# jfc4050/detect-to-track

Measured on AMD Instinct MI355X. Metric: PointwiseCorrelation fwd+bwd Gvox/s (and % HBM roofline) at B=8 C=256 38×63 d=8, higher is better.
Workload: dtype f32

## Files before the change

### detect-to-track_amd/csrc/d2t_corr_bwd8.hip

```cpp
#include "d2t_corr_common.hpp"
#include <type_traits>

namespace d2t { namespace tuned {

#ifdef D2T_LAB
__device__ unsigned long long* lab8_stamps;
#define D2T_WCLK(var) do { __builtin_amdgcn_sched_barrier(0); asm volatile("s_memtime %0\n\ts_waitcnt lgkmcnt(0)" : "=s"(var)::"memory"); __builtin_amdgcn_sched_barrier(0); } while (0)
#define D2T_WRT(var) do { __builtin_amdgcn_sched_barrier(0); asm volatile("s_memrealtime %0\n\ts_waitcnt lgkmcnt(0)" : "=s"(var)::"memory"); __builtin_amdgcn_sched_barrier(0); } while (0)
#define D2T_LAB_ONLY(...) __VA_ARGS__
#else
#define D2T_WCLK(var)
#define D2T_WRT(var)
#define D2T_LAB_ONLY(...)
#endif

namespace {

constexpr int S8_CH = 256;
constexpr int S8_QUADS = KB_SS * NACT * 64;
constexpr int S8_RING = 2048 * 4;
constexpr int S8_OOR = 0x7ffffff0;

struct Quad8 { int off, info; };

template <bool ROWKB>
__device__ __forceinline__ void kb_slot(int q, int gg, int& xr, int& cg)
{
    if (ROWKB) {
        xr = q < 4 ? q : gg;
        cg = q < 4 ? gg : 4;
    } else {
        const int x = 4 * q + gg;
        xr = (x * 13) >> 6;
        cg = x - xr * NCG;
    }
}

template <bool ROWKB>
__device__ __forceinline__ Quad8 quad8_desc(int role, int e, int H, int W, int tiles_i, int j0, int col0)
{
    const int q = e / (NACT * 64), r = e - q * (NACT * 64);
    const int a = r >> 6, l = r & 63, gg = l >> 4;
    int xr, cg;
    kb_slot<ROWKB>(q < KB_SS ? q : 0, gg, xr, cg);
    const int tpi = (l >> 2) & 3, lo2 = l & 3;
    const int ci = role ? 4 * a + tpi - xr : xr - 4 * a - tpi + 2 * DT;
    const int tj = j0 + lo2, sj = col0 + 4 * cg + (role ? lo2 : 0);
    const int cj = role ? j0 - sj + DT : sj - tj + DT;
    int mask = 0;
#pragma unroll
    for (int c = 0; c < 4; ++c) {
        const bool col_ok = role ? j0 + c < W : tj < W;
        mask |= (cj + c >= 0 && cj + c < 2 * DT && col_ok) ? (1 << c) : 0;
    }
    if (ci < 0 || ci >= 2 * DT || e >= S8_QUADS) mask = 0;
    const int pix0 = role ? xr * W + sj : (4 * (a - 2) + tpi) * W + tj;
    int lo = 2 - a, hi = tiles_i + 2 - a;
    const int hi_t = (H - tpi + 3) / 4 + 2 - a;
    const int hi_r = (H - xr + 3) / 4;
    hi = hi < hi_t ? hi : hi_t;
    hi = hi < hi_r ? hi : hi_r;
    lo = lo < 0 ? 0 : lo;
    if (!mask || hi < lo) { lo = 0; hi = 0; }
    Quad8 d;
    d.off = (pix0 * CELLS + ci * CW + cj) * 4;
    d.info = lo | (hi << 8) | (mask << 16);
    return d;
}

__device__ __forceinline__ f32x4 quad8_fix(const f32x4& v, int info)
{
    const u32x4 b = __builtin_bit_cast(u32x4, v);
    u32x4 o;
#pragma unroll
    for (int c = 0; c < 4; ++c) o[c] = b[c] & (unsigned)__builtin_amdgcn_sbfe(info, 16 + c, 1);
    return __builtin_bit_cast(f32x4, o);
}

typedef std::integral_constant<int, 0> I0;
typedef std::integral_constant<int, 1> I1;
typedef std::integral_constant<int, 2> I2;
typedef std::integral_constant<int, 3> I3;
typedef std::integral_constant<int, 4> I4;
typedef std::integral_constant<int, 5> I5;

#define D2T_PIN() __builtin_amdgcn_sched_barrier(0)

#ifndef D2T_EXP_GCO
#define D2T_EXP_GCO 1
#endif
#ifndef D2T_EXP_SWZ
#define D2T_EXP_SWZ 1
#endif
#ifndef D2T_EXP_PRIO
#define D2T_EXP_PRIO 0
#endif
#ifndef S8_ABL
#define S8_ABL 0
#endif
template <int role, int S8_CT, bool ROWKB, int ABL = 0, bool FLEX = false>
__device__ __forceinline__ void strip8_body(float (&ring)[2][S8_RING], const float* __restrict__ gout,
                                            const float* __restrict__ fm0, const float* __restrict__ fm1,
                                            float* __restrict__ g0, float* __restrict__ g1,
                                            int b, int tj, int C, int H, int W, int tiles_i, int ct0, int nct)
{
    constexpr int S8_WAVES = 16 / S8_CT;
    constexpr int GT = S8_WAVES * 64, S8_NQ = 2048 / GT;
    constexpr int DEAD0 = ROWKB ? 3 : KB_SS - 1;
    const int tid = threadIdx.x, lane = tid & 63, n = lane & 15, g = lane >> 4;
    const int wave = __builtin_amdgcn_readfirstlane(tid >> 6);
    D2T_LAB_ONLY(unsigned long long w_t0, w_t1, w_t2, w_t3, w_r1, w_r2, w_a, w_b, w_sl[3] = {0, 0, 0}, w_bar = 0, w_rot = 0;)
    D2T_WCLK(w_t0);
    const int j0 = tj * TP, HW = H * W;
    const int wleft = j0 - DT + role;
    const int col0 = wleft < 0 ? 0 : (wleft > W - WC ? W - WC : wleft);
    const float* S = (role ? fm0 : fm1) + (size_t)b * C * HW;
    float* gx = (role ? g1 : g0) + (size_t)b * C * HW;
    const float* gb = gout + (size_t)b * HW * CELLS;
    const unsigned plane_bytes = (unsigned)C * HW * 4u;
    const __amdgpu_buffer_rsrc_t rs = uniform_rsrc(S, plane_bytes);
    const __amdgpu_buffer_rsrc_t rx = uniform_rsrc(gx, plane_bytes);
    const __amdgpu_buffer_rsrc_t rg = uniform_rsrc(gb, (unsigned)HW * CELLS * 4u);

    const int cw = FLEX ? (ct0 + wave) * 16 : ct0 * 16 + wave * (S8_CT * 16);
    const bool on[2] = {!FLEX || wave < nct, !FLEX || wave + S8_WAVES < nct};
    int sv[KB_SS];
#pragma unroll
    for (int q = 0; q < KB_SS; ++q) {
        int xr, cg;
        kb_slot<ROWKB>(q, g, xr, cg);
        sv[q] = ((cw + n) * HW + xr * W + col0 + 4 * cg) * 4;
    }
    const int s_step = 4 * W * 4, ct_step = (FLEX ? S8_WAVES * 16 : 16) * HW * 4;
    auto s_load = [&](int ss, int q, int ct) -> f32x4 {
        const u32x4 v = __builtin_amdgcn_raw_buffer_load_b128(rs, sv[q] + ss * s_step + ct * ct_step, 0, 0);
        return __builtin_bit_cast(f32x4, v);
    };

    const int gtid = tid;
    constexpr bool GCO = D2T_EXP_GCO && ROWKB && role == 0;
    auto ring_index = [&](int ep) -> int {
        if (!GCO || ep >= S8_QUADS) return ep;
        const int p = (ep * 3277) >> 16, m = ep - p * 20;
        const int a = p >> 4, pix = p & 15, xr = (m * 13) >> 6, cg = m - xr * 5;
        const int q = cg < 4 ? xr : 4, gg = cg < 4 ? cg : xr;
        return (q * NACT + a) * 64 + gg * 16 + pix;
    };
    Quad8 qd[S8_NQ];
    int er[S8_NQ];
#pragma unroll
    for (int k = 0; k < S8_NQ; ++k) {
        er[k] = ring_index(gtid + k * GT);
        qd[k] = quad8_desc<ROWKB>(role, er[k], H, W, tiles_i, j0, col0);
    }
    const int g_step = 4 * W * CELLS * 4;
    auto g_load = [&](int k, int ss) -> f32x4 {
        const int lo = qd[k].info & 255, hi = (qd[k].info >> 8) & 255;
        const int v = ss >= lo && ss < hi ? qd[k].off + ss * g_step : S8_OOR;
        return __builtin_bit_cast(f32x4, __builtin_amdgcn_raw_buffer_load_b128(rg, v, 0, 0));
    };
    auto g_put = [&](float* rb, int k, const f32x4& raw) {
        const f32x4 v = quad8_fix(raw, qd[k].info);
        const int e = GCO ? er[k] : gtid + k * GT;
        const int f = D2T_EXP_SWZ ? (e >> 4) & 3 : 0;
        if (!role) { reinterpret_cast<f32x4*>(rb)[e ^ f] = v; return; }
        float* w = rb + (((e & ~63) + (lane & 0x3c)) << 2) + (lane & 3);
        w[(0 ^ f) << 2] = v[0]; w[(1 ^ f) << 2] = v[1]; w[(2 ^ f) << 2] = v[2]; w[(3 ^ f) << 2] = v[3];
    };
    f32x4 gn[S8_NQ];
    auto g_load_all = [&](int ss) {
#pragma unroll
        for (int k = 0; k < S8_NQ; ++k) gn[k] = g_load(k, ss);
    };
    auto g_put_all = [&](float* rb) {
#pragma unroll
        for (int k = 0; k < S8_NQ; ++k) g_put(rb, k, gn[k]);
    };

    unsigned long long badt = 0;
    const int x_lane = ((cw + 4 * g) * HW + (n >> 2) * W + j0 + (n & 3)) * 4;
    const bool col_ok = j0 + (n & 3) < W;
    auto store_tile = [&](const f32x4 (&d)[S8_CT], int u) {
        if (u < 0 || u >= tiles_i) return;
        const int i = 4 * u + (n >> 2);
        const int base = col_ok && i < H ? x_lane + 4 * u * W * 4 : S8_OOR;
        bool bad = false;
#pragma unroll
        for (int ct = 0; ct < S8_CT; ++ct) bad = bad || (on[ct] && nonfinite4(d[ct]));
        badt |= bad && base != S8_OOR ? 1ull << (u & 63) : 0ull;
#pragma unroll
        for (int ct = 0; ct < S8_CT; ++ct) {
            if (FLEX && !on[ct]) continue;
#pragma unroll
            for (int r = 0; r < 4; ++r) {
                const float v = d[ct][r];
                __builtin_amdgcn_raw_buffer_store_b32(__builtin_bit_cast(unsigned, v), rx,
                                                      base == S8_OOR ? S8_OOR : base + ct * ct_step + r * HW * 4, 0, 0);
            }
        }
    };

    f32x4 acc[S8_CT][NACT], a4[KB_SS][S8_CT], done[S8_CT];
#pragma unroll
    for (int ct = 0; ct < S8_CT; ++ct) {
        done[ct] = f32x4{0.f, 0.f, 0.f, 0.f};
#pragma unroll
        for (int a = 0; a < NACT; ++a) acc[ct][a] = f32x4{0.f, 0.f, 0.f, 0.f};
    }

    g_load_all(0);
#pragma unroll
    for (int q = 0; q < KB_SS; ++q)
#pragma unroll
        for (int ct = 0; ct < S8_CT; ++ct) a4[q][ct] = !FLEX || on[ct] ? s_load(0, q, ct) : f32x4{0.f, 0.f, 0.f, 0.f};
    g_put_all(ring[0]);
    g_load_all(1);
    lds_barrier();

    const f32x4* lane_ring = reinterpret_cast<const f32x4*>(&ring[0][0]) + (D2T_EXP_SWZ ? lane ^ (g & 3) : lane);
    f32x4 bvP[NACT], bvQ[NACT];
    auto b_fetch = [&](f32x4 (&bv)[NACT], int buf, int q, auto lo_c, auto hi_c) {
        constexpr int LO = decltype(lo_c)::value, HI = decltype(hi_c)::value;
#pragma unroll
        for (int a = LO; a < HI; ++a) bv[a] = lane_ring[buf * (S8_RING / 4) + (q * NACT + a) * 64];
    };

    auto super_step = [&](int ss, f32x4 (&bvC)[NACT], f32x4 (&bvN)[NACT], auto lo_c, auto hi_c, auto nlo_c, auto nhi_c) {
        constexpr int LO = decltype(lo_c)::value, HI = decltype(hi_c)::value;
        const int cur = ss & 1;
        auto mfma = [&](const f32x4 (&bv)[NACT], int q, int s_lo, int s_hi) {
            if (ROWKB && HI == NACT - 2 && q < 4 && 4 * ss + q >= H) return;
            const int A0 = (role == 0 && q == DEAD0 && LO == 0) ? 1 : LO;
            const int A1 = (role == 1 && q == 0 && HI == NACT) ? NACT - 1 : HI;
            if (!FLEX) {
#pragma unroll
                for (int s = s_lo; s < s_hi; ++s)
#pragma unroll
                    for (int a = A0; a < A1; ++a)
#pragma unroll
                        for (int ct = 0; ct < S8_CT; ++ct) acc[ct][a] = D2T_MFMA(a4[q][ct][s], bv[a][s], acc[ct][a]);
            } else {
#pragma unroll
                for (int ct = 0; ct < S8_CT; ++ct) {
                    if (!on[ct]) continue;
#pragma unroll
                    for (int s = s_lo; s < s_hi; ++s)
#pragma unroll
                        for (int a = A0; a < A1; ++a) acc[ct][a] = D2T_MFMA(a4[q][ct][s], bv[a][s], acc[ct][a]);
                }
            }
        };
        auto kblock = [&](f32x4 (&bv)[NACT], f32x4 (&bvn)[NACT], auto q_c) {
            constexpr int q = decltype(q_c)::value;
            mfma(bv, q, 0, 1);
            D2T_PIN();
            if (q + 1 < KB_SS) b_fetch(bvn, cur, q + 1, lo_c, hi_c);
            D2T_PIN();
            mfma(bv, q, 1, 2);
            D2T_PIN();
            auto slice = [&]() {
                if (q <= 2) D2T_WCLK(w_a);
                if (q == 0) {
                    if (!(ABL & 2)) store_tile(done, ss - 3);
                    else asm volatile("" ::"v"(done[0]), "v"(done[S8_CT - 1]));
                }
                if (q == 1 && !(ABL & 8)) g_put_all(ring[cur ^ 1]);
                if (q == 2 && !(ABL & 4)) g_load_all(ss + 2);
                if (q <= 2) { D2T_WCLK(w_b); D2T_LAB_ONLY(w_sl[q <= 2 ? q : 0] += w_b - w_a;) }
            };
            slice();
            D2T_PIN();
            mfma(bv, q, 2, 4);
            D2T_PIN();
#pragma unroll
            for (int ct = 0; ct < S8_CT; ++ct)
                if (!(ABL & 1) && (!FLEX || on[ct])) a4[q][ct] = s_load(ss + 1, q, ct);
            if (q == KB_SS - 2) {
                D2T_WCLK(w_a);
                lds_barrier();
                D2T_WCLK(w_b);
                D2T_LAB_ONLY(w_bar += w_b - w_a;)
                b_fetch(bv, cur ^ 1, 0, nlo_c, nhi_c);
            }
            D2T_PIN();
        };
        kblock(bvC, bvN, I0{});
        kblock(bvN, bvC, I1{});
        kblock(bvC, bvN, I2{});
        kblock(bvN, bvC, I3{});
        kblock(bvC, bvN, I4{});
        D2T_WCLK(w_a);
#pragma unroll
        for (int ct = 0; ct < S8_CT; ++ct) {
            done[ct] = acc[ct][0];
#pragma unroll
            for (int a = 0; a + 1 < NACT; ++a) acc[ct][a] = acc[ct][a + 1];
            acc[ct][NACT - 1] = f32x4{0.f, 0.f, 0.f, 0.f};
        }
        D2T_PIN();
        D2T_WCLK(w_b);
        D2T_LAB_ONLY(w_rot += w_b - w_a;)
    };

    b_fetch(bvP, 0, 0, I2{}, I5{});
#if D2T_EXP_PRIO
    if (wave >= S8_WAVES / 2) __builtin_amdgcn_s_setprio(1);
#endif
    D2T_WCLK(w_t1); D2T_WRT(w_r1);
    super_step(0, bvP, bvQ, I2{}, I5{}, I1{}, I5{});
    {
        super_step(1, bvQ, bvP, I1{}, I5{}, I0{}, I5{});
        int ss = 2;
        const int last_full = tiles_i - 3;
        for (; ss + 1 < last_full; ss += 2) {
            super_step(ss, bvP, bvQ, I0{}, I5{}, I0{}, I5{});
            super_step(ss + 1, bvQ, bvP, I0{}, I5{}, I0{}, I5{});
        }
        if (ss < last_full) {
            super_step(ss, bvP, bvQ, I0{}, I5{}, I0{}, I5{});
            super_step(ss + 1, bvQ, bvP, I0{}, I5{}, I0{}, I4{});
            super_step(ss + 2, bvP, bvQ, I0{}, I4{}, I0{}, I3{});
            super_step(ss + 3, bvQ, bvP, I0{}, I3{}, I0{}, I3{});
        } else {
            super_step(ss, bvP, bvQ, I0{}, I5{}, I0{}, I4{});
            super_step(ss + 1, bvQ, bvP, I0{}, I4{}, I0{}, I3{});
            super_step(ss + 2, bvP, bvQ, I0{}, I3{}, I0{}, I3{});
        }
    }
    D2T_WCLK(w_t2); D2T_WRT(w_r2);
    store_tile(done, tiles_i - 3);
    {
        f32x4 t0[S8_CT], t1[S8_CT];
#pragma unroll
        for (int ct = 0; ct < S8_CT; ++ct) { t0[ct] = acc[ct][0]; t1[ct] = acc[ct][1]; }
        store_tile(t0, tiles_i - 2);
        store_tile(t1, tiles_i - 1);
    }

#ifdef D2T_LAB
    asm volatile("s_waitcnt vmcnt(0)" ::: "memory");
    D2T_WCLK(w_t3);
    if (lane == 0) {
        unsigned long long* o = lab8_stamps + ((size_t)(blockIdx.x + gridDim.x * blockIdx.y) * S8_WAVES + wave) * 16;
        o[0] = w_t0; o[1] = w_t1; o[2] = w_t2; o[3] = w_t3; o[4] = w_r1; o[5] = w_r2; o[6] = w_sl[0]; o[7] = w_sl[1]; o[8] = w_sl[2];
        o[9] = w_bar; o[10] = w_rot;
    }
#endif
    if (__builtin_expect(__any(badt != 0), 0)) {
        unsigned lo = (unsigned)badt, hi = (unsigned)(badt >> 32);
#pragma unroll
        for (int off = 32; off; off >>= 1) { lo |= __shfl_xor(lo, off, 64); hi |= __shfl_xor(hi, off, 64); }
        const unsigned long long m = ((unsigned long long)hi << 32) | lo;
        for (int ct = 0; ct < S8_CT; ++ct) {
            if (FLEX && !on[ct]) continue;
            if (tiles_i > 64) {
                strip_repair(role, lane, gb, S, gx, cw + (FLEX ? 16 * S8_WAVES : 16) * ct, C, H, W, j0, CELLS, 1, 0, H);
            } else {
                for (int u = 0; u < tiles_i; ++u)
                    if ((m >> u) & 1)
                        strip_repair(role, lane, gb, S, gx, cw + (FLEX ? 16 * S8_WAVES : 16) * ct, C, H, W, j0, CELLS, 1, 4 * u, 4 * u + 4 < H ? 4 * u + 4 : H);
            }
        }
    }
}
#undef D2T_PIN

template <int CT, bool ROWKB, int ABL = 0, bool FLEX = false>
__global__ void __launch_bounds__(1024 / CT)
k_corr_bwd_strip8(const float* __restrict__ gout, const float* __restrict__ fm0, const float* __restrict__ fm1,
                  float* __restrict__ g0, float* __restrict__ g1,
                  int B, int C, int H, int W, int tiles_i, int tiles_j)
{
    __shared__ __attribute__((aligned(16))) float ring[2][S8_RING];
    const int nb = gridDim.y, lid = xcd_remap(blockIdx.x + gridDim.x * blockIdx.y, gridDim.x * nb);
    const int tj = lid % tiles_j, yb = (lid / tiles_j) % nb, role = (lid / (tiles_j * nb)) & 1, b = lid / (2 * tiles_j * nb);
    const int Ct = (C + 15) / 16;
    const int ct0 = FLEX ? (int)((long long)yb * Ct / nb) : 16 * yb;
    const int nct = FLEX ? (int)((long long)(yb + 1) * Ct / nb) - ct0 : 16;
    if ((S8_ABL & 32) && role) return;
    if ((S8_ABL & 64) && !role) return;
    if (role) strip8_body<1, CT, ROWKB, ABL, FLEX>(ring, gout, fm0, fm1, g0, g1, b, tj, C, H, W, tiles_i, ct0, nct);
    else strip8_body<0, CT, ROWKB, ABL, FLEX>(ring, gout, fm0, fm1, g0, g1, b, tj, C, H, W, tiles_i, ct0, nct);
}

}

bool corr_bwd8_supported(int B, int C, int H, int W, int ps, int cs)
{
    if (ps != CELLS || cs != 1 || B < 1 || C < 1 || W < WC) return false;
    const int tiles_i = (H + TP - 1) / TP;
    if (tiles_i < 5 || tiles_i > 250) return false;
    const bool fits = (C + 64LL) * H * W * 4 + 64LL * W < 0x7ffffff0LL && (1LL * H * W + 8LL * W) * CELLS * 4 < 0x7ffffff0LL;
    return fits && 2LL * B * ((W + TP - 1) / TP) * ((C + S8_CH - 1) / S8_CH) <= 0x7fffffffLL;
}

#ifdef D2T_LAB
template <int ABL>
void lab8_launch(const float* gout, const float* fm0, const float* fm1, float* g0, float* g1, int B, int C, int H, int W)
{
    const int tiles_i = (H + TP - 1) / TP, tiles_j = (W + TP - 1) / TP;
    hipLaunchKernelGGL((k_corr_bwd_strip8<2, true, ABL>), dim3(2 * B * tiles_j, (C + S8_CH - 1) / S8_CH), dim3(512), 0, 0,
                       gout, fm0, fm1, g0, g1, B, C, H, W, tiles_i, tiles_j);
}
#endif

int corr_bwd8_blocks(int B, int C, int W)
{
    const int Ct = (C + 15) / 16, strips = 2 * B * ((W + TP - 1) / TP);
    int best = (Ct + 15) / 16;
    double best_t = 1e30;
    for (int nb = (Ct + 15) / 16; nb <= Ct && nb <= 64; ++nb) {
        const int n = (Ct + nb - 1) / nb, per_simd = (n + 3) / 4;
        const long long wgs = 1LL * strips * nb;
        const double t = (double)((wgs + 255) / 256) * (12.0 + 15.0 * per_simd);
        if (t < best_t - 1e-9) { best_t = t; best = nb; }
    }
    return best;
}

int corr_bwd8_f32(const float* gout, const float* fm0, const float* fm1, float* g0, float* g1,
                  int B, int C, int H, int W, hipStream_t st, int variant)
{
    const int tiles_i = (H + TP - 1) / TP, tiles_j = (W + TP - 1) / TP;
    const int nb = corr_bwd8_blocks(B, C, W);
    if (variant == 1) {
        hipLaunchKernelGGL((k_corr_bwd_strip8<2, false>), dim3(2 * B * tiles_j, (C + S8_CH - 1) / S8_CH), dim3(512), 0, st,
                           gout, fm0, fm1, g0, g1, B, C, H, W, tiles_i, tiles_j);
    } else if (C % S8_CH == 0 && nb == C / S8_CH) {
        hipLaunchKernelGGL((k_corr_bwd_strip8<2, true, (S8_ABL & 15)>), dim3(2 * B * tiles_j, nb), dim3(512), 0, st,
                           gout, fm0, fm1, g0, g1, B, C, H, W, tiles_i, tiles_j);
    } else {
        hipLaunchKernelGGL((k_corr_bwd_strip8<2, true, 0, true>), dim3(2 * B * tiles_j, nb), dim3(512), 0, st,
                           gout, fm0, fm1, g0, g1, B, C, H, W, tiles_i, tiles_j);
    }
    return launch_status();
}

}}
```

### lab/csrc/bwd8_stamp_lab.hip

```cpp
#define D2T_LAB 1
#include "../../detect-to-track_amd/csrc/d2t_corr_bwd8.hip"
#include <algorithm>
#include <cstdio>
#include <vector>

using namespace d2t::tuned;

static double med(std::vector<double> v) { std::sort(v.begin(), v.end()); return v[v.size() / 2]; }

int main(int argc, char** argv)
{
    const int B = argc > 1 ? atoi(argv[1]) : 8, C = argc > 2 ? atoi(argv[2]) : 256, H = 38, W = argc > 3 ? atoi(argv[3]) : 63;
    const int NS = 4, iters = 200;
    const size_t nin = (size_t)B * C * H * W, nout = (size_t)B * H * W * 289;
    std::vector<float> h(nin), hg(nout);
    for (size_t i = 0; i < nin; ++i) h[i] = (float)((i * 2654435761u >> 8) & 0xffff) / 65536.f;
    for (size_t i = 0; i < nout; ++i) hg[i] = (float)((i * 40503u >> 4) & 0xffff) / 65536.f;
    float *f0[NS], *f1[NS], *go[NS], *g0[NS], *g1[NS];
    for (int s = 0; s < NS; ++s) {
        hipMalloc(&f0[s], nin * 4); hipMalloc(&f1[s], nin * 4); hipMalloc(&go[s], nout * 4);
        hipMalloc(&g0[s], nin * 4); hipMalloc(&g1[s], nin * 4);
        hipMemcpy(f0[s], h.data(), nin * 4, hipMemcpyHostToDevice);
        hipMemcpy(f1[s], h.data(), nin * 4, hipMemcpyHostToDevice);
        hipMemcpy(go[s], hg.data(), nout * 4, hipMemcpyHostToDevice);
    }
    const int tiles_j = (W + 3) / 4;
    const int blocks = 2 * B * tiles_j * ((C + 255) / 256), NW = 8;
    unsigned long long* st;
    hipMalloc(&st, (size_t)blocks * NW * 16 * 8);
    hipMemset(st, 0, (size_t)blocks * NW * 16 * 8);
    hipMemcpyToSymbol(HIP_SYMBOL(lab8_stamps), &st, sizeof(st));
    typedef void (*launch_t)(const float*, const float*, const float*, float*, float*, int, int, int, int);
    const launch_t abl[] = {lab8_launch<0>, lab8_launch<1>, lab8_launch<2>, lab8_launch<4>, lab8_launch<12>, lab8_launch<6>, lab8_launch<7>, lab8_launch<15>};
    const char* abl_name[] = {"all in", "no S reloads", "no tile stores", "no G loads", "no G loads, no ring writes", "no stores, no G loads", "no S, no stores, no G loads", "MFMA + LDS reads + barriers only"};
    {
        hipEvent_t a, b; hipEventCreate(&a); hipEventCreate(&b);
        for (int rnd = 0; rnd < 3; ++rnd)
            for (int v = 0; v < 8; ++v) {
                for (int i = 0; i < NS; ++i) abl[v](go[i], f0[i], f1[i], g0[i], g1[i], B, C, H, W);
                hipEventRecord(a);
                for (int i = 0; i < 100; ++i) abl[v](go[i % NS], f0[i % NS], f1[i % NS], g0[i % NS], g1[i % NS], B, C, H, W);
                hipEventRecord(b); hipEventSynchronize(b);
                float ms; hipEventElapsedTime(&ms, a, b);
                printf("round %d  %-36s %.1f us\n", rnd, abl_name[v], ms * 10.f);
            }
    }
    auto run = [&](int i) { abl[0](go[i % NS], f0[i % NS], f1[i % NS], g0[i % NS], g1[i % NS], B, C, H, W); };
    for (int i = 0; i < 2 * NS; ++i) run(i);
    hipDeviceSynchronize();
    hipEvent_t a, b; hipEventCreate(&a); hipEventCreate(&b);
    hipEventRecord(a);
    for (int i = 0; i < iters; ++i) run(i);
    hipEventRecord(b); hipEventSynchronize(b);
    float ms; hipEventElapsedTime(&ms, a, b);
    printf("B=%d C=%d %dx%d: %d workgroups, %.1f us per launch (stamped build)\n", B, C, H, W, blocks, ms * 1000.f / iters);
    std::vector<unsigned long long> s((size_t)blocks * NW * 16);
    hipMemcpy(s.data(), st, s.size() * 8, hipMemcpyDeviceToHost);
    const char* names[] = {"prologue (descriptors, S + G(0), barrier)", "loop", "final stores + drain", "  slice: tile store", "  slice: ring put",
                           "  slice: G load issue", "  barrier wait", "  rotate", "shader clock in the loop (MHz)"};
    for (int role = 0; role < 2; ++role) {
        std::vector<double> v[9], tot;
        for (int w = 0; w < blocks; ++w) {
            const int xcd = w & 7, qq = blocks >> 3, rr = blocks & 7;
            const int bid = (xcd < rr ? xcd * (qq + 1) : rr * (qq + 1) + (xcd - rr) * qq) + (w >> 3);
            if (((bid / tiles_j) & 1) != role) continue;
            for (int k = 0; k < NW; ++k) {
                const unsigned long long* p = &s[((size_t)w * NW + k) * 16];
                v[0].push_back((double)(p[1] - p[0])); v[1].push_back((double)(p[2] - p[1])); v[2].push_back((double)(p[3] - p[2]));
                for (int j = 0; j < 5; ++j) v[3 + j].push_back((double)p[6 + j]);
                v[8].push_back((double)(p[2] - p[1]) / (double)(p[5] - p[4]) * 100.0);
                tot.push_back((double)(p[3] - p[0]));
            }
        }
        printf("role %d (median over waves, shader clock cycles)\n", role);
        for (int k = 0; k < 9; ++k) printf("  %-44s %9.0f\n", names[k], med(v[k]));
        printf("  %-44s %9.0f\n", "wave total", med(tot));
    }
    for (int w = 40; w < 42; ++w) {
        printf("workgroup %d: barrier wait by wave:", w);
        for (int k = 0; k < NW; ++k) printf(" %llu", s[((size_t)w * NW + k) * 16 + 9]);
        printf("\n");
    }
    return 0;
}
```

Before: 50.49.

## Reorder role-1 gradient ring layout and specialize tail loop on tile parity

```diff
diff --git a/detect-to-track_amd/csrc/d2t_corr_bwd8.hip b/detect-to-track_amd/csrc/d2t_corr_bwd8.hip
--- a/detect-to-track_amd/csrc/d2t_corr_bwd8.hip
+++ b/detect-to-track_amd/csrc/d2t_corr_bwd8.hip
@@ -8,6 +8,7 @@
 #define D2T_WCLK(var) do { __builtin_amdgcn_sched_barrier(0); asm volatile("s_memtime %0\n\ts_waitcnt lgkmcnt(0)" : "=s"(var)::"memory"); __builtin_amdgcn_sched_barrier(0); } while (0)
 #define D2T_WRT(var) do { __builtin_amdgcn_sched_barrier(0); asm volatile("s_memrealtime %0\n\ts_waitcnt lgkmcnt(0)" : "=s"(var)::"memory"); __builtin_amdgcn_sched_barrier(0); } while (0)
 #define D2T_LAB_ONLY(...) __VA_ARGS__
+#define D2T_SCLK(ptr) do { unsigned long long t_; __builtin_amdgcn_sched_barrier(0); asm volatile("s_memtime %0\n\ts_waitcnt lgkmcnt(0)\n\ts_store_dwordx2 %0, %1, 0x0" : "=&s"(t_) : "s"(ptr) : "memory"); __builtin_amdgcn_sched_barrier(0); } while (0)
 #else
 #define D2T_WCLK(var)
 #define D2T_WRT(var)
@@ -89,6 +90,9 @@
 #ifndef D2T_EXP_GCO
 #define D2T_EXP_GCO 1
 #endif
+#ifndef D2T_EXP_GCO1
+#define D2T_EXP_GCO1 1
+#endif
 #ifndef D2T_EXP_SWZ
 #define D2T_EXP_SWZ 1
 #endif
@@ -98,7 +102,7 @@
 #ifndef S8_ABL
 #define S8_ABL 0
 #endif
-template <int role, int S8_CT, bool ROWKB, int ABL = 0, bool FLEX = false>
+template <int role, int S8_CT, bool ROWKB, int ABL = 0, bool FLEX = false, bool ODD = false>
 __device__ __forceinline__ void strip8_body(float (&ring)[2][S8_RING], const float* __restrict__ gout,
                                             const float* __restrict__ fm0, const float* __restrict__ fm1,
                                             float* __restrict__ g0, float* __restrict__ g1,
@@ -111,6 +115,7 @@
     const int wave = __builtin_amdgcn_readfirstlane(tid >> 6);
     D2T_LAB_ONLY(unsigned long long w_t0, w_t1, w_t2, w_t3, w_r1, w_r2, w_a, w_b, w_sl[3] = {0, 0, 0}, w_bar = 0, w_rot = 0;)
     D2T_WCLK(w_t0);
+    D2T_LAB_ONLY(unsigned long long* const w_ss = lab8_stamps + ((size_t)(blockIdx.x + gridDim.x * blockIdx.y) * S8_WAVES + wave) * 32 + 16;)
     const int j0 = tj * TP, HW = H * W;
     const int wleft = j0 - DT + role;
     const int col0 = wleft < 0 ? 0 : (wleft > W - WC ? W - WC : wleft);
@@ -138,9 +143,16 @@
     };
 
     const int gtid = tid;
-    constexpr bool GCO = D2T_EXP_GCO && ROWKB && role == 0;
+    constexpr bool GCO1 = D2T_EXP_GCO1 && ROWKB && role == 1 && D2T_EXP_SWZ;
+    constexpr bool GCO = (D2T_EXP_GCO && ROWKB && role == 0) || GCO1;
     auto ring_index = [&](int ep) -> int {
         if (!GCO || ep >= S8_QUADS) return ep;
+        if (GCO1) {
+            const int p = (ep * 3277) >> 16, m = ep - p * 20;
+            const int lo2 = p & 3, t = p >> 2, xr = (t * 13) >> 6, cg = t - xr * 5;
+            const int q = cg < 4 ? xr : 4, gg = cg < 4 ? cg : xr;
+            return (q * NACT + (m >> 2)) * 64 + gg * 16 + (m & 3) * 4 + lo2;
+        }
         const int p = (ep * 3277) >> 16, m = ep - p * 20;
         const int a = p >> 4, pix = p & 15, xr = (m * 13) >> 6, cg = m - xr * 5;
         const int q = cg < 4 ? xr : 4, gg = cg < 4 ? cg : xr;
@@ -159,12 +171,14 @@
         const int v = ss >= lo && ss < hi ? qd[k].off + ss * g_step : S8_OOR;
         return __builtin_bit_cast(f32x4, __builtin_amdgcn_raw_buffer_load_b128(rg, v, 0, 0));
     };
+    auto rs_f = [](int u) -> int { return ((u & 3) + (u >> 2) % NACT) & 3; };
     auto g_put = [&](float* rb, int k, const f32x4& raw) {
         const f32x4 v = quad8_fix(raw, qd[k].info);
         const int e = GCO ? er[k] : gtid + k * GT;
-        const int f = D2T_EXP_SWZ ? (e >> 4) & 3 : 0;
+        const int f = !D2T_EXP_SWZ ? 0 : GCO1 ? rs_f(e >> 4) : (e >> 4) & 3;
         if (!role) { reinterpret_cast<f32x4*>(rb)[e ^ f] = v; return; }
-        float* w = rb + (((e & ~63) + (lane & 0x3c)) << 2) + (lane & 3);
+        const int l = GCO1 ? e & 63 : lane;
+        float* w = rb + (((e & ~63) + (l & 0x3c)) << 2) + (l & 3);
         w[(0 ^ f) << 2] = v[0]; w[(1 ^ f) << 2] = v[1]; w[(2 ^ f) << 2] = v[2]; w[(3 ^ f) << 2] = v[3];
     };
     f32x4 gn[S8_NQ];
@@ -218,16 +232,21 @@
     lds_barrier();
 
     const f32x4* lane_ring = reinterpret_cast<const f32x4*>(&ring[0][0]) + (D2T_EXP_SWZ ? lane ^ (g & 3) : lane);
+    const f32x4* lane_ring1[4];
+#pragma unroll
+    for (int r = 0; r < 4; ++r) lane_ring1[r] = reinterpret_cast<const f32x4*>(&ring[0][0]) + (lane ^ ((g + r) & 3));
     f32x4 bvP[NACT], bvQ[NACT];
     auto b_fetch = [&](f32x4 (&bv)[NACT], int buf, int q, auto lo_c, auto hi_c) {
         constexpr int LO = decltype(lo_c)::value, HI = decltype(hi_c)::value;
 #pragma unroll
-        for (int a = LO; a < HI; ++a) bv[a] = lane_ring[buf * (S8_RING / 4) + (q * NACT + a) * 64];
+        for (int a = LO; a < HI; ++a)
+            bv[a] = (GCO1 ? lane_ring1[a & 3] : lane_ring)[buf * (S8_RING / 4) + (q * NACT + a) * 64];
     };
 
     auto super_step = [&](int ss, f32x4 (&bvC)[NACT], f32x4 (&bvN)[NACT], auto lo_c, auto hi_c, auto nlo_c, auto nhi_c) {
         constexpr int LO = decltype(lo_c)::value, HI = decltype(hi_c)::value;
         const int cur = ss & 1;
+        D2T_LAB_ONLY(if (ss < 16) D2T_SCLK(w_ss + ss);)
         auto mfma = [&](const f32x4 (&bv)[NACT], int q, int s_lo, int s_hi) {
             if (ROWKB && HI == NACT - 2 && q < 4 && 4 * ss + q >= H) return;
             const int A0 = (role == 0 && q == DEAD0 && LO == 0) ? 1 : LO;
@@ -316,7 +335,7 @@
             super_step(ss, bvP, bvQ, I0{}, I5{}, I0{}, I5{});
             super_step(ss + 1, bvQ, bvP, I0{}, I5{}, I0{}, I5{});
         }
-        if (ss < last_full) {
+        if constexpr (!ODD) {
             super_step(ss, bvP, bvQ, I0{}, I5{}, I0{}, I5{});
             super_step(ss + 1, bvQ, bvP, I0{}, I5{}, I0{}, I4{});
             super_step(ss + 2, bvP, bvQ, I0{}, I4{}, I0{}, I3{});
@@ -341,10 +360,11 @@
     asm volatile("s_waitcnt vmcnt(0)" ::: "memory");
     D2T_WCLK(w_t3);
     if (lane == 0) {
-        unsigned long long* o = lab8_stamps + ((size_t)(blockIdx.x + gridDim.x * blockIdx.y) * S8_WAVES + wave) * 16;
+        unsigned long long* o = lab8_stamps + ((size_t)(blockIdx.x + gridDim.x * blockIdx.y) * S8_WAVES + wave) * 32;
         o[0] = w_t0; o[1] = w_t1; o[2] = w_t2; o[3] = w_t3; o[4] = w_r1; o[5] = w_r2; o[6] = w_sl[0]; o[7] = w_sl[1]; o[8] = w_sl[2];
         o[9] = w_bar; o[10] = w_rot;
     }
+    asm volatile("s_dcache_wb" ::: "memory");
 #endif
     if (__builtin_expect(__any(badt != 0), 0)) {
         unsigned lo = (unsigned)badt, hi = (unsigned)(badt >> 32);
@@ -365,7 +385,7 @@
 }
 #undef D2T_PIN
 
-template <int CT, bool ROWKB, int ABL = 0, bool FLEX = false>
+template <int CT, bool ROWKB, int ABL = 0, bool FLEX = false, bool ODD = false>
 __global__ void __launch_bounds__(1024 / CT)
 k_corr_bwd_strip8(const float* __restrict__ gout, const float* __restrict__ fm0, const float* __restrict__ fm1,
                   float* __restrict__ g0, float* __restrict__ g1,
@@ -379,8 +399,8 @@
     const int nct = FLEX ? (int)((long long)(yb + 1) * Ct / nb) - ct0 : 16;
     if ((S8_ABL & 32) && role) return;
     if ((S8_ABL & 64) && !role) return;
-    if (role) strip8_body<1, CT, ROWKB, ABL, FLEX>(ring, gout, fm0, fm1, g0, g1, b, tj, C, H, W, tiles_i, ct0, nct);
-    else strip8_body<0, CT, ROWKB, ABL, FLEX>(ring, gout, fm0, fm1, g0, g1, b, tj, C, H, W, tiles_i, ct0, nct);
+    if (role) strip8_body<1, CT, ROWKB, ABL, FLEX, ODD>(ring, gout, fm0, fm1, g0, g1, b, tj, C, H, W, tiles_i, ct0, nct);
+    else strip8_body<0, CT, ROWKB, ABL, FLEX, ODD>(ring, gout, fm0, fm1, g0, g1, b, tj, C, H, W, tiles_i, ct0, nct);
 }
 
 }
@@ -399,8 +419,11 @@
 void lab8_launch(const float* gout, const float* fm0, const float* fm1, float* g0, float* g1, int B, int C, int H, int W)
 {
     const int tiles_i = (H + TP - 1) / TP, tiles_j = (W + TP - 1) / TP;
-    hipLaunchKernelGGL((k_corr_bwd_strip8<2, true, ABL>), dim3(2 * B * tiles_j, (C + S8_CH - 1) / S8_CH), dim3(512), 0, 0,
-                       gout, fm0, fm1, g0, g1, B, C, H, W, tiles_i, tiles_j);
+    const dim3 grid(2 * B * tiles_j, (C + S8_CH - 1) / S8_CH);
+    if (tiles_i & 1)
+        hipLaunchKernelGGL((k_corr_bwd_strip8<2, true, ABL, false, true>), grid, dim3(512), 0, 0, gout, fm0, fm1, g0, g1, B, C, H, W, tiles_i, tiles_j);
+    else
+        hipLaunchKernelGGL((k_corr_bwd_strip8<2, true, ABL>), grid, dim3(512), 0, 0, gout, fm0, fm1, g0, g1, B, C, H, W, tiles_i, tiles_j);
 }
 #endif
 
@@ -418,21 +441,29 @@
     return best;
 }
 
+template <bool ROWKB, int ABL, bool FLEX>
+void launch_bwd8(dim3 grid, hipStream_t st, const float* gout, const float* fm0, const float* fm1, float* g0, float* g1,
+                 int B, int C, int H, int W, int tiles_i, int tiles_j)
+{
+    if (tiles_i & 1)
+        hipLaunchKernelGGL((k_corr_bwd_strip8<2, ROWKB, ABL, FLEX, true>), grid, dim3(512), 0, st,
+                           gout, fm0, fm1, g0, g1, B, C, H, W, tiles_i, tiles_j);
+    else
+        hipLaunchKernelGGL((k_corr_bwd_strip8<2, ROWKB, ABL, FLEX, false>), grid, dim3(512), 0, st,
+                           gout, fm0, fm1, g0, g1, B, C, H, W, tiles_i, tiles_j);
+}
+
 int corr_bwd8_f32(const float* gout, const float* fm0, const float* fm1, float* g0, float* g1,
                   int B, int C, int H, int W, hipStream_t st, int variant)
 {
     const int tiles_i = (H + TP - 1) / TP, tiles_j = (W + TP - 1) / TP;
     const int nb = corr_bwd8_blocks(B, C, W);
-    if (variant == 1) {
-        hipLaunchKernelGGL((k_corr_bwd_strip8<2, false>), dim3(2 * B * tiles_j, (C + S8_CH - 1) / S8_CH), dim3(512), 0, st,
-                           gout, fm0, fm1, g0, g1, B, C, H, W, tiles_i, tiles_j);
-    } else if (C % S8_CH == 0 && nb == C / S8_CH) {
-        hipLaunchKernelGGL((k_corr_bwd_strip8<2, true, (S8_ABL & 15)>), dim3(2 * B * tiles_j, nb), dim3(512), 0, st,
-                           gout, fm0, fm1, g0, g1, B, C, H, W, tiles_i, tiles_j);
-    } else {
-        hipLaunchKernelGGL((k_corr_bwd_strip8<2, true, 0, true>), dim3(2 * B * tiles_j, nb), dim3(512), 0, st,
-                           gout, fm0, fm1, g0, g1, B, C, H, W, tiles_i, tiles_j);
-    }
+    if (variant == 1)
+        launch_bwd8<false, 0, false>(dim3(2 * B * tiles_j, (C + S8_CH - 1) / S8_CH), st, gout, fm0, fm1, g0, g1, B, C, H, W, tiles_i, tiles_j);
+    else if (C % S8_CH == 0 && nb == C / S8_CH)
+        launch_bwd8<true, (S8_ABL & 15), false>(dim3(2 * B * tiles_j, nb), st, gout, fm0, fm1, g0, g1, B, C, H, W, tiles_i, tiles_j);
+    else
+        launch_bwd8<true, 0, true>(dim3(2 * B * tiles_j, nb), st, gout, fm0, fm1, g0, g1, B, C, H, W, tiles_i, tiles_j);
     return launch_status();
 }
 
diff --git a/lab/csrc/bwd8_stamp_lab.hip b/lab/csrc/bwd8_stamp_lab.hip
--- a/lab/csrc/bwd8_stamp_lab.hip
+++ b/lab/csrc/bwd8_stamp_lab.hip
@@ -27,8 +27,10 @@
     const int tiles_j = (W + 3) / 4;
     const int blocks = 2 * B * tiles_j * ((C + 255) / 256), NW = 8;
     unsigned long long* st;
-    hipMalloc(&st, (size_t)blocks * NW * 16 * 8);
-    hipMemset(st, 0, (size_t)blocks * NW * 16 * 8);
+    const int NSL = 32, tiles_i = (H + 3) / 4;
+    if (tiles_i > 15) { printf("super-step stamps need tiles_i <= 15\n"); return 1; }
+    hipMalloc(&st, (size_t)blocks * NW * NSL * 8);
+    hipMemset(st, 0, (size_t)blocks * NW * NSL * 8);
     hipMemcpyToSymbol(HIP_SYMBOL(lab8_stamps), &st, sizeof(st));
     typedef void (*launch_t)(const float*, const float*, const float*, float*, float*, int, int, int, int);
     const launch_t abl[] = {lab8_launch<0>, lab8_launch<1>, lab8_launch<2>, lab8_launch<4>, lab8_launch<12>, lab8_launch<6>, lab8_launch<7>, lab8_launch<15>};
@@ -54,7 +56,7 @@
     hipEventRecord(b); hipEventSynchronize(b);
     float ms; hipEventElapsedTime(&ms, a, b);
     printf("B=%d C=%d %dx%d: %d workgroups, %.1f us per launch (stamped build)\n", B, C, H, W, blocks, ms * 1000.f / iters);
-    std::vector<unsigned long long> s((size_t)blocks * NW * 16);
+    std::vector<unsigned long long> s((size_t)blocks * NW * NSL);
     hipMemcpy(s.data(), st, s.size() * 8, hipMemcpyDeviceToHost);
     const char* names[] = {"prologue (descriptors, S + G(0), barrier)", "loop", "final stores + drain", "  slice: tile store", "  slice: ring put",
                            "  slice: G load issue", "  barrier wait", "  rotate", "shader clock in the loop (MHz)"};
@@ -65,7 +67,7 @@
             const int bid = (xcd < rr ? xcd * (qq + 1) : rr * (qq + 1) + (xcd - rr) * qq) + (w >> 3);
             if (((bid / tiles_j) & 1) != role) continue;
             for (int k = 0; k < NW; ++k) {
-                const unsigned long long* p = &s[((size_t)w * NW + k) * 16];
+                const unsigned long long* p = &s[((size_t)w * NW + k) * NSL];
                 v[0].push_back((double)(p[1] - p[0])); v[1].push_back((double)(p[2] - p[1])); v[2].push_back((double)(p[3] - p[2]));
                 for (int j = 0; j < 5; ++j) v[3 + j].push_back((double)p[6 + j]);
                 v[8].push_back((double)(p[2] - p[1]) / (double)(p[5] - p[4]) * 100.0);
@@ -78,8 +80,34 @@
     }
     for (int w = 40; w < 42; ++w) {
         printf("workgroup %d: barrier wait by wave:", w);
-        for (int k = 0; k < NW; ++k) printf(" %llu", s[((size_t)w * NW + k) * 16 + 9]);
+        for (int k = 0; k < NW; ++k) printf(" %llu", s[((size_t)w * NW + k) * NSL + 9]);
         printf("\n");
+    }
+    printf("per super-step (median over waves, shader clock cycles; MFMAs issued by one wave; cycles per MFMA)\n");
+    for (int role = 0; role < 2; ++role) {
+        printf("role %d\n", role);
+        for (int ss = 0; ss < tiles_i; ++ss) {
+            const int LO = ss == 0 ? 2 : ss == 1 ? 1 : 0, HI = ss == tiles_i - 1 ? 3 : ss == tiles_i - 2 ? 4 : 5;
+            int mf = 0;
+            for (int q = 0; q < 5; ++q) {
+                if (HI == 3 && q < 4 && 4 * ss + q >= H) continue;
+                const int A0 = (role == 0 && q == 3 && LO == 0) ? 1 : LO, A1 = (role == 1 && q == 0 && HI == 5) ? 4 : HI;
+                mf += (A1 - A0) * 4 * 2;
+            }
+            std::vector<double> v;
+            for (int w = 0; w < blocks; ++w) {
+                const int xcd = w & 7, qq = blocks >> 3, rr = blocks & 7;
+                const int bid = (xcd < rr ? xcd * (qq + 1) : rr * (qq + 1) + (xcd - rr) * qq) + (w >> 3);
+                if (((bid / tiles_j) & 1) != role) continue;
+                for (int k = 0; k < NW; ++k) {
+                    const unsigned long long* p = &s[((size_t)w * NW + k) * NSL];
+                    const unsigned long long e = ss + 1 < tiles_i ? p[16 + ss + 1] : p[2];
+                    v.push_back((double)(e - p[16 + ss]));
+                }
+            }
+            const double m = med(v);
+            printf("  super-step %2d  live tiles [%d,%d)  %8.0f cycles  %4d MFMAs  %6.1f cycles / MFMA\n", ss, LO, HI, m, mf, m / mf);
+        }
     }
     return 0;
 }
```

New measurement: 50.41, median of 6. Within noise of the previous version (-0.2%).
